# aleksgri/3D-wave-equation-MPI-CUDA

Hardware: AMD Instinct MI355X
Metric: Mpoints/sec (whole node) + L∞ error vs analytic, N=512³ fp64 (higher is better)
Workload: dtype fp64; 1 GPU; model=wave3d leapfrog 7-point, N=512^3, L=pi, T=1, timesteps=100, global_batch=1, seq_len=513, parallelism=dd1x1x1-tb4, N=512, kernel=tb4, overlap=False, overlap_mode=none, overlap_order=none, transport=self, hip_graph=True, device_bytes_per_gpu=4742168192

## Files before the change

3d-wave-equation-mpi-cuda_amd/csrc/hip_kernels.hip:

```cpp
#include <hip/hip_runtime.h>

#include <cstdlib>

#include <algorithm>

#include "device_common.hpp"


namespace wave3d {
namespace {

template <class T>
struct StepParams {
    int xcd;
    int delta;
    const T* u1;
    const T* u2;
    T* u;
    T* dout;
    i64 si;
    int sj;
    int poff;
    int jmax, kmax;
    int nbox;
// ... 342 lines not shown
    if (j <= bx.j1) {
        const T tyj = ty[j];
        bool nz = false, any = false;
        for (int i = ib; i <= ie; ++i) {
            const T txi = tx[i];
            const i64 row = i64(j) * sj;
            for (int k = bx.k0 + lane; k <= bx.k1; k += 64) {
                const T f = analytic(txi, tyj, tz[k], ct);
                u[i64(i) * si + row + k] = f;
#pragma unroll
                for (int q = 0; q < kMaxWrap; ++q)
                    if (i == wrap.src[q]) u[i64(wrap.dst[q]) * si + row + k] = f;
                chk += f;
                nz |= f != T(0);
                any = true;
            }
        }
        if (any) ma = T(0);
        if (nz) mr = T(0);
    }
    commit_errors(ma, mr, chk, err);
}

template <class T>
__global__ void k_zero_faces(T* u, i64 si, int sj, int X, int Y, int Z, int G, int mask) {
    const int i = 1 - G + blockIdx.y;
    const int t = 1 + blockIdx.x * blockDim.x + threadIdx.x;
    T* pl = u + i64(i) * si;
    if (t <= Y) {
        if (mask & 1) pl[t * sj + 1] = T(0);
        if (mask & 2) pl[t * sj + Z] = T(0);
    }
    if (t <= Z) {
        if (mask & 4) pl[1 * sj + t] = T(0);
        if (mask & 8) pl[Y * sj + t] = T(0);
    }
}

template <class T>
struct FaceOps {
    FaceOp<T> op[4];
};

template <class T>
__global__ void k_faces(T* u, i64 si, int sj, int ny, int nz, FaceOps<T> ops, bool to_buf) {
    const FaceOp<T> f = ops.op[blockIdx.z];
// ... 61 lines not shown
    return v.march && !v.flat ? kWaves * v.rows : kNaiveTJ;
}

int tile_order() {
    static const int order = [] {
        const char* e = std::getenv("WAVE3D_TILE_ORDER");
        const std::string v = e ? e : "";
        if (v == "k") return 0;
        if (v == "j") return 1;
        if (v == "blocks") return 3;
        W3D_REQUIRE(v.empty() || v == "band", "WAVE3D_TILE_ORDER must be band, blocks, j or k, not " + v);
        return 2;
    }();
    return order;
}

bool xcd_swizzle_enabled() {
    static const bool on = [] {
        const char* e = std::getenv("WAVE3D_XCD_SWIZZLE");
        return e && e[0] == '1';
    }();
    return on;
}

KernelVariant parse_kernel_variant(const std::string& name) {
    KernelVariant v;
    if (name == "naive") {
        v.march = false;
        return v;
    }
    if (name == "flat") {
        v.march = false, v.flat = true;
        return v;
    }
    if (name == "auto") {
        v.rows = 4;
        v.nt = true;
        return v;
    }
    W3D_REQUIRE(name.rfind("march", 0) == 0, "wave3d: unknown kernel variant " + name);
    std::string s = name.substr(5);
    if (!s.empty() && (s[0] == '2' || s[0] == '4' || s[0] == '8')) v.rows = s[0] - '0', s = s.substr(1);
    if (s == "nt") v.nt = true;
    else if (s == "f") v.fast = true;
    else if (s == "p") v.pk = true;
    else W3D_REQUIRE(s.empty(), "wave3d: unknown kernel variant " + name);
// ... 128 lines not shown
        L.block_begin = total;
        total += L.tiles_k * L.tiles_j * cdiv(planes, ch);
        ++nb;
    }
    p.nbox = nb;
    if (nb == 0) return;
    void (*kern)(const StepParams<T>);
    if (march) kern = first ? march_kernel<T, true>(kind) : march_kernel<T, false>(kind);
    else kern = first ? k_naive<T, true> : k_naive<T, false>;
    hipLaunchKernelGGL(kern, dim3(total), dim3(kThreads), 0, s, p);
    HIP_OK(hipGetLastError());
}

template <class T>
void launch_init(T* u, const GridView& gv, const Box& bx, const Wrap& wrap, const T* tx,
                 const T* ty, const T* tz, double ct0, u64* err, hipStream_t s) {
    if (bx.empty()) return;
    W3D_REQUIRE(bx.i0 >= 1 && bx.i1 <= gv.X && bx.j1 <= gv.Y && bx.k1 <= gv.Z,
                "init box outside the owned region");
    const int planes = bx.i1 - bx.i0 + 1;
    const int rowblocks = cdiv(bx.j1 - bx.j0 + 1, kWaves);
    const int chunk = std::min(planes, std::max(1, cdiv(planes * rowblocks, 4096)));
    dim3 grid(rowblocks, cdiv(planes, chunk));
    hipLaunchKernelGGL(k_init<T>, grid, dim3(kThreads), 0, s, u, gv.si, gv.sj, bx, chunk, wrap, tx,
                       ty, tz, T(ct0), err);
    HIP_OK(hipGetLastError());
}

template <class T>
void launch_zero_faces(T* u, const GridView& gv, int mask, hipStream_t s) {
    if (!mask) return;
    dim3 grid(cdiv(std::max(gv.Y, gv.Z), 256), gv.X + 2 * gv.G);
    hipLaunchKernelGGL(k_zero_faces<T>, grid, dim3(256), 0, s, u, gv.si, gv.sj, gv.X, gv.Y, gv.Z,
                       gv.G, mask);
    HIP_OK(hipGetLastError());
}

template <class T>
void launch_faces(T* u, const GridView& gv, const FaceOp<T>* ops, int nops, bool to_buf,
                  hipStream_t s) {
    W3D_REQUIRE(nops <= 4, "too many faces");
    if (nops <= 0) return;
    FaceOps<T> f{};
    for (int q = 0; q < nops; ++q) f.op[q] = ops[q];
    const int len = std::max(gv.Y, gv.Z) + 2;
    dim3 grid(cdiv(len, 256), gv.X, nops);
    hipLaunchKernelGGL(k_faces<T>, grid, dim3(256), 0, s, u, gv.si, gv.sj, gv.Y + 2, gv.Z + 2, f,
                       to_buf);
// ... 118 lines not shown
```

3d-wave-equation-mpi-cuda_amd/csrc/hip_kernels.hpp:

```cpp
#pragma once

#include <hip/hip_runtime.h>

#include <string>

#include "common.hpp"

namespace wave3d {

struct GridView {
    int X = 0, Y = 0, Z = 0;
    int G = 1;
    int sj = 0;
    i64 si = 0;
    int poff = 0;
    int jmax() const { return Y + G; }
    int kmax() const { return Z + G; }
};

constexpr int kMaxBoxes = 7;
constexpr int kTileK = 64;

struct StepCoefs {
    double hx2 = 1, hy2 = 1, hz2 = 1;
// ... 46 lines not shown
    int axis = 1;
    int index = 0;
};
template <class T>
void launch_faces(T* u, const GridView& gv, const FaceOp<T>* ops, int nops, bool to_buf,
                  hipStream_t s);

template <class T>
struct SeamPartners {
    int next_i = -(1 << 30), prev_i = -(1 << 30);
    const T *nA = nullptr, *nC = nullptr;
    const T *pA = nullptr, *pC = nullptr;
};
template <class T>
struct SeamCPlane {
    T* out = nullptr;
    const T *Ac = nullptr, *Am = nullptr, *Ap = nullptr, *Bc = nullptr;
    T* dout = nullptr;
};
constexpr int kMaxSeamOps = 6;
template <class T>
void launch_seam_c(bool first, bool delta, bool fm, const SeamCPlane<T>* ops, int nops, const GridView& gv,
                   const Box& cdom, const StepCoefs& cC, hipStream_t s);
bool tb3_supported(int rows, int waves, bool fm = false);
bool tb3_delta_supported(int rows, int waves, bool fm = false);
template <class T>
void launch_tb3(int rows, int waves, bool delta, bool fm, bool first, const T* A, const T* B, T* D, T* E,
                const GridView& gv, const Box* boxes, int nbox, const Box& cdom, int ei0, int ei1,
                const Wrap& wrapD, const Wrap& wrapE, const SeamPartners<T>& seam, const T* txy,
                const T* tz, const T* txr, const T* rtz, const StepCoefs& cC, const StepCoefs& cD,
                const StepCoefs& cE, u64* errC, u64* errD, u64* errE, int chunk, hipStream_t s);

constexpr int kTbnMaxDepth = 4;
template <class T>
struct TbnSeam {
    int next_i = -(1 << 30), prev_i = -(1 << 30);
    const T* nP[kTbnMaxDepth - 1] = {};
    const T* pP[kTbnMaxDepth - 1] = {};
};
bool tbn_supported(int depth, int rows, int waves, bool fm, bool fp32);
bool tbn_delta_supported(int depth, int rows, int waves, bool fm, bool fp32);
template <class T>
void launch_tbn(int depth, int rows, int waves, bool fm, bool first, const T* A, const T* B, T* O0, T* O1,
                const GridView& gv, const Box* boxes, int nbox, const Box& cdom, int ei0, int ei1,
                const Wrap& wrap0, const Wrap& wrap1, const TbnSeam<T>& seam, const T* txy, const T* tz,
                const T* txr, const T* rtz, const StepCoefs* c, u64* const* err, int chunk, hipStream_t s,
// ... 36 lines not shown
```

3d-wave-equation-mpi-cuda_amd/csrc/hip_solver.hip:

```cpp
#include <hip/hip_runtime.h>

#include <algorithm>
#include <chrono>
#include <cstdlib>
#include <cstring>
#include <iostream>
#include <map>
#include <memory>
#include <thread>

#include "checkpoint.hpp"
#include "device_common.hpp"
#include "hip_kernels.hpp"
#include "hip_selftest.hpp"
#include "rccl_transport.hpp"
#include "problem.hpp"
#include "sizing.hpp"
#include "solver.hpp"
#include "log.hpp"
#include "trace.hpp"

#define HIP_CHECK(x)                                                                   \
    do {                                                                               \
        hipError_t e_ = (x);                                                           \
// ... 62 lines not shown
        int peer, tag;
        int level;
        Box box;
        T* buf;
    };
    std::vector<BoxMsg> tb_bsends[2], tb_brecvs[2];
    std::vector<BoxMsg> tb_dsends, tb_drecvs;
    struct PeerBuf {
        int peer;
        T* buf;
        size_t count;
    };
    std::vector<PeerBuf> tb_psends, tb_precvs;
    struct PipeGroup {
        std::vector<PlaneMsg> sends, recvs;
        std::vector<BoxMsg> dsends, drecvs;
        std::vector<PeerBuf> psends, precvs;
    };
    std::vector<PipeGroup> pipe;
    std::vector<Box> slabs;
    T* alias[2][2] = {};
    T* seamc_buf = nullptr;
    T* seamc_in = nullptr;
    T* pinned = nullptr;
    Box tb_interior;
    std::vector<Box> tb_shell;
};

constexpr int kAliasPlane = -1000;

template <class T>
class HipSolver {
public:
    HipSolver(const Config& c, Transport* ext) : cfg_(c), ext_(ext) {
        prob_ = Problem::from_config(c);
        fault_ = FaultSpec::parse(c.fault);
        if (ext_) {
            W3D_REQUIRE(ext_->device(), "run_hip needs a device transport");
            world_ = ext_->size();
            local_ = {ext_->rank()};
        } else {
            world_ = std::max(1, c.ranks);
            for (int r = 0; r < world_; ++r) local_.push_back(r);
        }
        const Layout lay = plan_layout(c, world_);
        tb_ = lay.tb;
// ... 1035 lines not shown
            const T* cXp = op(c_ops, 2, Ap(X + 1), Ap(1), Ap(X + 2), Bp(X + 1));
            sp.next_i = 0, sp.nP[0] = Ap(X), sp.nP[1] = cX, sp.nP[2] = op(d_ops, 6, cX, cXm, cXp, dpl(8, Ap(X)));
            const T* c1 = op(c_ops, 3, Ap(1), Ap(0), Ap(2), Bp(1), 9);
            const T* c0 = op(c_ops, 4, Ap(0), Ap(-1), Ap(X), Bp(0));
            const T* c2 = op(c_ops, 5, Ap(2), Ap(1), Ap(3), Bp(2));
            sp.prev_i = X + 1, sp.pP[0] = Ap(1), sp.pP[1] = c1, sp.pP[2] = op(d_ops, 7, c1, c0, c2, dpl(9, Ap(1)));
        } else if (R.topo.first(0)) {
            const T* cN = op(c_ops, 0, aA, Ap(0), Ap(2), aB, 8);
            const T* cNm = op(c_ops, 1, Ap(0), Ap(-1), aA, Bp(0));
            const T* c1 = op(c_ops, 2, Ap(2), Ap(1), Ap(3), Bp(2));
            sp.next_i = 0, sp.nP[0] = aA, sp.nP[1] = cN, sp.nP[2] = op(d_ops, 6, cN, cNm, c1, dpl(8, aA));
        } else if (R.topo.last(0)) {
            const T* c0 = op(c_ops, 3, aA, Ap(X - 1), Ap(X + 1), aB, 9);
            const T* cm = op(c_ops, 4, Ap(X - 1), Ap(X - 2), Ap(X), Bp(X - 1));
            const T* cp = op(c_ops, 5, Ap(X + 1), aA, Ap(X + 2), Bp(X + 1));
            sp.prev_i = X + 1, sp.pP[0] = aA, sp.pP[1] = c0, sp.pP[2] = op(d_ops, 7, c0, cm, cp, dpl(9, aA));
        }
        return sp;
    }

    void seam4(DevRank<T>& R, int m, hipStream_t s) {
        std::vector<SeamCPlane<T>> c_ops, d_ops;
        seam_partners4(R, m, &c_ops, &d_ops);
        launch_seam_c<T>(m == 1, cfg_.delta, cfg_.fma, c_ops.data(), int(c_ops.size()), R.gv, R.cdom, coefs(m), s);
        launch_seam_c<T>(false, cfg_.delta, cfg_.fma, d_ops.data(), int(d_ops.size()), R.gv, R.cdom, coefs(m + 1), s);
    }

    void sweep4(DevRank<T>& R, int m, hipStream_t s, const Box* boxes = nullptr, int nbox = 0) {
        const T* A = R.g[lvl(m - 1)];
        const T* B = R.g[lvl(m - 2)];
        const TbnSeam<T> sp = seam_partners4(R, m, nullptr, nullptr);
        if (!boxes) boxes = &R.compute, nbox = 1;
        StepCoefs c[4];
        u64* err[4];
        for (int l = 0; l < 4; ++l) c[l] = coefs(m + l), err[l] = R.err + size_t(m + l) * kSlotsPerLayer;
        launch_tbn<T>(4, tb_rows_, tb_waves_, cfg_.fma, m == 1, A, B, R.g[lvl(m + 2)], R.g[lvl(m + 3)], R.gv, boxes,
                      nbox, R.cdom, R.error.i0, R.error.i1, R.wrap3, R.wrap4, sp, R.txy, R.tz, R.rtxy, R.rtz, c,
                      err, cfg_.chunk, s, cfg_.delta);
    }

    void seam_pre(DevRank<T>& R, int m, int span, hipStream_t s, bool in = false) {
        SeamScratch use(R, in);
        if (span == 4) seam4(R, m, s);
        else seam_c(R, m, s);
    }
    void sweep_deep(DevRank<T>& R, int m, int span, hipStream_t s, const Box* boxes = nullptr, int nbox = 0,
// ... 475 lines not shown
            launch_init<T>(R.g[lvl(0)], R.gv, R.owned, wrap_depth(R, G_), R.tx, R.ty, R.tz, ct_[0],
                           R.err, s_comp_);
            pack_faces(R, 0, s_comp_, true);
        }
        mark(s_comp_, 1);
        if (prob_.K >= 1) issue_exchange(0);
    }

    int enqueue_layers(RunResult& res, int start) {
        TraceRange tr("wave3d.layers");
        order_enqueued_ = !overlap_ ? "none" : pipe_ ? "pipe" : shells_first_ ? "shells_first" : "beside";
        pipe_prev_ = false;
        CuReserveScope cu_scope(s_comp_ == s_comp_cu_ ? comm_cus_ : 0);
        const int K = prob_.K;
        int done = start - 1;
        for (int n = start; n <= K;) {
            const int span = span_at(n);
            bool comm_follows = false;
            for (int q = n; q < n + span; ++q) guard_checkpoint_level(lvl(q), s_comp_);
            if (cfg_.delta && span == 1 && n > 1) guard_checkpoint_level(dlvl(n - 1), s_comp_);
            if (cfg_.print_layers && !cfg_.quiet && !capturing_ && ranks_[0].topo.rank == 0)
                for (int q = n; q < n + span; ++q) std::cout << "calculating layer " << q << "\n";
            mark(s_comp_, 0);
            for (int q = n; q < n + span; ++q)
                for (auto& R : ranks_)
                    if ((first_write_[q + 1] || q == start) && !(span >= 3 && q < n + span - 2))
                        launch_zero_faces<T>(R.g[lvl(q)], R.gv, R.zero_mask, s_comp_);
            bool exchanged = false;
            if (span >= 3 && overlap_ && pipe_) {
                pipe_sweep(n, span, n + span - 1 < K);
                exchanged = true;
            } else if (span >= 3 && overlap_ && shells_first_) {
                HIP_CHECK(hipStreamWaitEvent(s_comp_, ev_halo_, 0));
                for (auto& R : ranks_) {
                    seam_pre(R, n, span, s_comp_);
                    if (!R.tb_shell.empty())
                        sweep_deep(R, n, span, s_comp_, R.tb_shell.data(), int(R.tb_shell.size()));
                }
                const int last = n + span - 1;
                if (last < K) {
                    HIP_CHECK(hipEventRecord(ev_shell_, s_comp_));
                    HIP_CHECK(hipStreamWaitEvent(s_comm_, ev_shell_, 0));
                    issue_exchange(last, true);
                    exchanged = true;
                }
                for (auto& R : ranks_)
                    if (!R.tb_interior.empty()) sweep_deep(R, n, span, s_comp_, &R.tb_interior, 1);
            } else if (span >= 3 && overlap_) {
                HIP_CHECK(hipEventRecord(ev_layer_, s_comp_));
                HIP_CHECK(hipStreamWaitEvent(s_comm_, ev_layer_, 0));
// ... 428 lines not shown
```

3d-wave-equation-mpi-cuda_amd/csrc/hip_tb3.hip:

```cpp
#include <hip/hip_runtime.h>

#include <algorithm>
#include <climits>
#include <cmath>
#include <type_traits>

#include "device_common.hpp"

namespace wave3d {
namespace {

template <class T>
struct Tb3Params {
    const char* A;
    const char* B;
    char* D;
    char* E;
    unsigned pbytes;
    int pbias;
    int order;
    int sj;
    int poff;
    int jmin, jmax, kmin, kmax;
    int cj0, cj1, ck0, ck1;
// ... 540 lines not shown
    };
    commit_errors<T, NW>(ma1, rel(mr1, 0), chk1, p.errC);
    __syncthreads();
    commit_errors<T, NW>(ma2, rel(mr2, 1), chk2, p.errD);
    __syncthreads();
    commit_errors<T, NW>(ma3, rel(mr3, 2), chk3, p.errE);
}

template <class T>
struct SeamCOp {
    T* out;
    const T *Ac, *Am, *Ap, *Bc;
    T* dout;
};
template <class T>
struct SeamCParams {
    SeamCOp<T> op[kMaxSeamOps];
    int sj, jmin, jmax, kmin, kmax;
    int cj0, cj1, ck0, ck1;
    T hx2, hy2, hz2, yx2, yy2, yz2, coef;
    T fc[3];
};

template <class T, bool FIRST, bool DELTA, bool FM>
__global__ void __launch_bounds__(kThreads) k_seam_c(const SeamCParams<T> p) {
    const SeamCOp<T> o = p.op[blockIdx.y];
    const int ktiles = (p.kmax - p.kmin - 1 + kTK - 1) / kTK;
    const int j = p.jmin + 1 + (int(blockIdx.x) / ktiles) * kWaves + int(threadIdx.x >> 6);
    const int k = p.kmin + 1 + (int(blockIdx.x) % ktiles) * kTK + int(threadIdx.x & 63);
    if (j > p.jmax - 1 || k > p.kmax - 1) return;
    const i64 c = i64(j) * p.sj + k;
    T v = T(0), d = T(0);
    if (j >= p.cj0 && j <= p.cj1 && k >= p.ck0 && k <= p.ck1) {
        const T a = o.Ac[c];
        if constexpr (FM) {
            const T l = coef_lap_fma(a, o.Am[c], o.Ap[c], o.Ac[c - p.sj], o.Ac[c + p.sj], o.Ac[c - 1], o.Ac[c + 1],
                                     p.fc[0], p.fc[1], p.fc[2]);
            if constexpr (DELTA)
                d = FIRST ? l : o.Bc[c] + l, v = a + d;
            else if constexpr (FIRST)
                v = a + l;
            else
                v = leap_fm(a, o.Bc[c], o.Am[c], o.Ap[c], o.Ac[c - p.sj], o.Ac[c + p.sj], o.Ac[c - 1], o.Ac[c + 1],
                            p.fc[0], p.fc[1], p.fc[2], fm_kc(p.fc[0], p.fc[1], p.fc[2]));
        } else {
            const T lap = laplace7_cr(a, o.Am[c], o.Ap[c], o.Ac[c - p.sj], o.Ac[c + p.sj], o.Ac[c - 1],
                                      o.Ac[c + 1], p.hx2, p.hy2, p.hz2, p.yx2, p.yy2, p.yz2);
            if constexpr (DELTA)
                d = FIRST ? p.coef * lap : delta_incr(o.Bc[c], lap, p.coef), v = a + d;
            else
                v = FIRST ? taylor_first(a, lap, p.coef) : leapfrog(a, o.Bc[c], lap, p.coef);
        }
    }
    o.out[c] = v;
    if (DELTA && o.dout) o.dout[c] = d;
}

template <class T, bool F>
static void (*tb3_kernel(int rows, int waves, bool fm = false))(const Tb3Params<T>) {
    if (fm) {
        switch (rows * 100 + waves) {
            case 208: return k_tb3<T, F, 2, 8, false, true>;
            case 108: return k_tb3<T, F, 1, 8, false, true>;
            case 116: return k_tb3<T, F, 1, 16, false, true>;
            default: return nullptr;
        }
    }
    switch (rows * 100 + waves) {
        case 404: return k_tb3<T, F, 4, 4>;
        case 208: return k_tb3<T, F, 2, 8>;
        case 204: return k_tb3<T, F, 2, 4>;
        case 116: return k_tb3<T, F, 1, 16>;
        case 108: return k_tb3<T, F, 1, 8>;
        default: return nullptr;
    }
}

}
// ... 112 lines not shown
                   const Box& cdom, const StepCoefs& cC, hipStream_t s) {
    W3D_REQUIRE(nops >= 0 && nops <= kMaxSeamOps, "seam C: too many planes");
    if (nops == 0) return;
    SeamCParams<T> p{};
    for (int q = 0; q < nops; ++q)
        p.op[q] = SeamCOp<T>{ops[q].out, ops[q].Ac, ops[q].Am, ops[q].Ap, ops[q].Bc ? ops[q].Bc : ops[q].Ac, ops[q].dout};
    p.sj = gv.sj;
    p.jmin = 1 - gv.G, p.jmax = gv.jmax(), p.kmin = 1 - gv.G, p.kmax = gv.kmax();
    p.cj0 = cdom.j0, p.cj1 = cdom.j1, p.ck0 = cdom.k0, p.ck1 = cdom.k1;
    p.hx2 = T(cC.hx2), p.hy2 = T(cC.hy2), p.hz2 = T(cC.hz2);
    p.yx2 = T(1) / T(cC.hx2), p.yy2 = T(1) / T(cC.hy2), p.yz2 = T(1) / T(cC.hz2);
    p.coef = T(cC.coef);
    fma_coefs(cC, p.fc);
    const int rows = p.jmax - p.jmin - 1, ktiles = cdiv(p.kmax - p.kmin - 1, kTK);
    const dim3 grid(cdiv(rows, kWaves) * ktiles, nops);
    void (*kern)(const SeamCParams<T>) =
        fm ? (delta ? (first ? k_seam_c<T, true, true, true> : k_seam_c<T, false, true, true>)
                    : (first ? k_seam_c<T, true, false, true> : k_seam_c<T, false, false, true>))
           : (delta ? (first ? k_seam_c<T, true, true, false> : k_seam_c<T, false, true, false>)
                    : (first ? k_seam_c<T, true, false, false> : k_seam_c<T, false, false, false>));
    hipLaunchKernelGGL(kern, grid, dim3(kThreads), 0, s, p);
    HIP_OK(hipGetLastError());
}
template void launch_seam_c<double>(bool, bool, bool, const SeamCPlane<double>*, int, const GridView&, const Box&,
                                    const StepCoefs&, hipStream_t);
template void launch_seam_c<float>(bool, bool, bool, const SeamCPlane<float>*, int, const GridView&, const Box&,
                                   const StepCoefs&, hipStream_t);

#define W3D_TB3_INST(T)                                                                       \
    template void launch_tb3<T>(int, int, bool, bool, bool, const T*, const T*, T*, T*, const GridView&, \
                                const Box*, int, const Box&, int, int, const Wrap&,           \
                                const Wrap&, const SeamPartners<T>&, const T*,                \
                                const T*, const T*, const T*, const StepCoefs&, const StepCoefs&, \
                                const StepCoefs&, u64*, u64*, u64*, int, hipStream_t);
W3D_TB3_INST(double)
W3D_TB3_INST(float)

}
```

3d-wave-equation-mpi-cuda_amd/csrc/hip_tbn.hip:

```cpp
#include <hip/hip_runtime.h>

#include <algorithm>
#include <climits>
#include <cstdlib>
#include <cmath>
#include <type_traits>
#include <utility>

#include "device_common.hpp"

#ifndef W3D_TBN_ABL_ERR
#define W3D_TBN_ABL_ERR 0
#endif

#ifndef W3D_TBN_PART
#define W3D_TBN_PART 1
#endif
#ifndef W3D_TBN_BOUND
#define W3D_TBN_BOUND 0
#endif
#ifndef W3D_TBN_MERGE
#define W3D_TBN_MERGE 1
#endif
#ifndef W3D_TBN_PRE
#define W3D_TBN_PRE 1
#endif
#ifndef W3D_TBN_DENSE
#define W3D_TBN_DENSE 1
#endif

namespace wave3d {
template <class T>
const void* tbn_exact_kernel(int depth, bool first, bool delta);

namespace {

template <class F, int... I>
__device__ __forceinline__ void sfor_impl(F&& f, std::integer_sequence<int, I...>) {
    (f(std::integral_constant<int, I>{}), ...);
}
template <int N, class F>
__device__ __forceinline__ void sfor(F&& f) {
    sfor_impl(f, std::make_integer_sequence<int, N>{});
}
template <int V>
using Ic = std::integral_constant<int, V>;

template <class T>
struct TbnParams {
    const char* A;
    const char* B;
// ... 34 lines not shown
    static constexpr int scells = RPW * NW * W(0);
    static constexpr int bcells = RPW * NW * W(1);
    static constexpr int rowb = (kTK + 2 * D) * ES;
    static constexpr int browb = (kTK + 2 * D - 2) * ES;
    static constexpr int bat(int y, int x) { return y * W(1) + x - 1; }
    static constexpr int a_off(int q) { return q * scells; }
    static constexpr int b_off(int q) { return 4 * scells + q * bcells; }
    static constexpr int u_off(int s, int h) {
        return s == 1 ? b_off(2) + h * cells(1) : u_off(s - 1, 1) + cells(s - 1) + h * cells(s);
    }
    static constexpr int total = u_off(D - 1, 1) + cells(D - 1);
    static constexpr int npos(int r) {
        return 2 * (kTK + 2 * (r - 1)) + 2 * (TJ + 2 * (r - (r == D - 1 ? 1 : 0)));
    }
    static constexpr int first(int r) { return r <= 1 ? 0 : first(r - 1) + npos(r - 1); }
    static constexpr int ncomp = first(D);
    static constexpr int ring_of(int q) {
        int r = 1;
        while (r < D && q >= first(r + 1)) ++r;
        return r;
    }
};

template <int W, int ROWS, int NW>
struct DenseDma {
    static constexpr int pitch = W * 8, pay = pitch - 8;
    static constexpr int chunks = ((ROWS - 1) * pitch + pay + 15) / 16;
    static constexpr int PW = (chunks + 64 * NW - 1) / (64 * NW);
    static constexpr int NP = NW * PW;
    static constexpr int L = (chunks + NP - 1) / NP;
    static constexpr int last = chunks - (NP - 1) * L;
    static constexpr int src_row(int c) { return 16 * c / pitch + (16 * c % pitch == pay ? 1 : 0); }
    static constexpr int src_col(int c) { return 16 * c % pitch == pay ? -1 : 16 * c % pitch / 8; }
    static constexpr bool covers() {
        if (W % 2 == 0 || last < 1 || L > 64 || 2 * chunks < (ROWS - 1) * W + W - 1) return false;
        for (int c = 0; c < chunks; ++c)
            for (int h = 0; h < 2; ++h) {
                const int y = (2 * c + h) / W, x = (2 * c + h) % W;
                if (y >= ROWS) return false;
                if (x < W - 1 && (src_row(c) != y || src_col(c) + h != x)) return false;
            }
        return true;
    }
};
template <int D>
constexpr bool dense_dma_ok() {
    using Gm = TbnGeom<D, 16, 8, 8>;
    return DenseDma<Gm::W(0), Gm::H(0), 8>::covers() && DenseDma<Gm::W(1), Gm::H(0) - 2, 8>::covers();
}
static_assert(dense_dma_ok<4>() && dense_dma_ok<3>(), "dense LDS-DMA cover of the A / B frames");
static_assert(DenseDma<73, 24, 8>::chunks == 876 && DenseDma<71, 22, 8>::chunks == 781 && DenseDma<73, 24, 8>::PW == 2 &&
                  DenseDma<71, 22, 8>::PW == 2,
              "D = 4: 2 + 2 pieces per wave");

template <class T>
__device__ __forceinline__ unsigned lds_addr(T* ptr) {
    return static_cast<unsigned>(reinterpret_cast<uintptr_t>((__attribute__((address_space(3))) T*)ptr));
}
template <int ES, int ROWB, int RB>
__device__ __forceinline__ void dma_fill3(__amdgpu_buffer_rsrc_t r, unsigned src0, unsigned sjb, unsigned slot,
                                          unsigned lds0) {
    unsigned v0, v1, v2;
    u64 keep;
    const unsigned lane = __builtin_amdgcn_mbcnt_hi(~0u, __builtin_amdgcn_mbcnt_lo(~0u, 0u));
    if constexpr (ES == 8) {
        static_assert(RB % 16 == 0 && RB <= 1024, "fp64 rows: one dwordx4 piece per lane");
        asm volatile(
            "s_add_u32 m0, %[slot], %[lds0]\n\t"
            "v_add_u32 %[v0], %[src0], %[l16]\n\t"
            "v_add_u32 %[v1], %[sjb], %[v0]\n\t"
            "v_add_u32 %[v2], %[sjb], %[v1]\n\t"
            "s_mov_b64 %[keep], exec\n\t"
            "s_mov_b64 exec, %[mask]\n\t"
            "buffer_load_dwordx4 %[v0], %[rs], 0 offen lds\n\t"
            "s_add_u32 m0, m0, %[rowb]\n\t"
            "s_nop 0\n\t"
// ... 210 lines not shown
    unsigned ra_off[RP];
    bool rcd[RP];
    int ry[RP], rx[RP];
#pragma unroll
    for (int s = 0; s < RP; ++s) {
        const int q = threadIdx.x + s * NT;
        int g = 0, rj = jt, rk = kb;
#pragma unroll
        for (int d = 1; d < D; ++d)
            if (g == 0 && q < Gm::first(d + 1)) {
                g = d;
                ring(d, d == D - 1 ? 1 : 0, q - Gm::first(d), rj, rk);
            }
        rg[s] = g;
        ry[s] = rj - jt + D, rx[s] = rk - kb + D;
        ro0[s] = Gm::at(0, ry[s], rx[s]);
        rb0[s] = Gm::bat(ry[s], rx[s]);
        rcd[s] = g != 0 && incd(rj, rk);
        ra_off[s] = boff(rj, rk, g != 0 && inb(rj, rk));
    }

    constexpr bool DENSE = W3D_TBN_DENSE && ES == 8;
    using DA = DenseDma<W0, Gm::H(0), NW>;
    using DB = DenseDma<Gm::W(1), Gm::H(0) - 2, NW>;
    static_assert(DENSE || Gm::RPW == 3, "dma_fill3: three slot rows per wave");
    static_assert(!DENSE || (DA::PW == 2 && DB::PW == 2 && DA::covers() && DB::covers()),
                  "dma_dense2: two pieces per wave and fill");
    const unsigned sjb = unsigned(sj) * ES;
    const unsigned src0 = unsigned((jt - D + (DENSE ? 0 : w * Gm::RPW)) * sj + kb - D + p.poff) * ES;
    const unsigned lds0 = unsigned(DENSE ? w * 2 * DA::L * 16 : w * Gm::RPW * W0 * ES);
    const unsigned bds0 = unsigned(DENSE ? w * 2 * DB::L * 16 + Gm::W(1) * ES : w * Gm::RPW * Gm::W(1) * ES);
    auto dsrc = [&](auto geom, int q, unsigned origin) {
        using Dn = decltype(geom);
        const int c = min((w * Dn::PW + q) * Dn::L + lane, Dn::chunks - 1);
        return origin + unsigned(Dn::src_row(c)) * sjb + unsigned(Dn::src_col(c) * ES);
    };
    const unsigned da0 = DENSE ? dsrc(DA{}, 0, src0) : 0u, da1 = DENSE ? dsrc(DA{}, 1, src0) : 0u;
    const unsigned db0 = DENSE ? dsrc(DB{}, 0, src0 + sjb + ES) : 0u, db1 = DENSE ? dsrc(DB{}, 1, src0 + sjb + ES) : 0u;
    const unsigned nla = w == NW - 1 ? DA::last : DA::L, nlb = w == NW - 1 ? DB::last : DB::L;
    auto fillA = [&](auto qc, int plane, bool live) {
        const auto rs = prs(p.A, plane, live ? pbytes : 0u);
        if constexpr (DENSE) dma_dense2<DA::L, DA::L * 16>(rs, da0, da1, nla, lds_addr(Ap(qc)), lds0);
        else dma_fill3<ES, W0 * ES, Gm::rowb>(rs, src0, sjb, lds_addr(Ap(qc)), lds0);
    };
    auto fillB = [&](int q, int plane, bool live) {
        const auto rs = prs(p.B, plane, live ? pbytes : 0u);
        const unsigned slot = __builtin_amdgcn_readfirstlane(lds_addr(Bp(q)));
        if constexpr (DENSE) dma_dense2<DB::L, DB::L * 16>(rs, db0, db1, nlb, slot, bds0);
        else dma_fill3<ES, Gm::W(1) * ES, Gm::browb>(rs, src0 + ES, sjb, slot, bds0);
    };
    constexpr int NST = 2 * R;
    constexpr int PA = DENSE ? DA::PW : (ES == 8 ? 1 : 2) * Gm::RPW, PB = DENSE ? DB::PW : PA;
    constexpr bool PRE = W3D_TBN_PRE && ES == 8 && FM && !DELTA;
    constexpr int NPRE = std::min(2 + 3 * R + 5 * RP, 15);
    constexpr int NDMA = PA + (FIRST ? 0 : PB);
    fillA(Ic<3>{}, i0 - 1, true);
    fillA(Ic<0>{}, i0, true);
    fillA(Ic<1>{}, i0 + 1, true);
    fillA(Ic<2>{}, i0 + 2, true);
    if constexpr (!FIRST) fillB(0, i0, true);
    vm_wait<0>();
    __syncthreads();
// ... 512 lines not shown
```

Baseline: 624,900 Mpoints/s.

## Vectorize init kernel, fuse seam planes with face zeroing, rebalance B-frame DMA

Adds a 16-byte vectorized init kernel that caches tz values and writes whole vectors per lane. Adds a fused seam4 kernel that computes the layer-m seam planes and the layer-m+1 plane in one launch, using an LDS ring for neighbors, and folds the pending face-zeroing work into the same grid. Also changes the dense LDS-DMA split of the B frame so three waves load one piece and the rest load two. These changes aim to cut launch count and load imbalance, at the cost of redundant recomputation of layer-m values at tile halos and more complex indexing.

```diff
diff --git a/3d-wave-equation-mpi-cuda_amd/csrc/hip_kernels.hip b/3d-wave-equation-mpi-cuda_amd/csrc/hip_kernels.hip
--- a/3d-wave-equation-mpi-cuda_amd/csrc/hip_kernels.hip
+++ b/3d-wave-equation-mpi-cuda_amd/csrc/hip_kernels.hip
@@ -388,6 +388,76 @@
     commit_errors(ma, mr, chk, err);
 }
 
+constexpr int kInitQ = 5;
+constexpr int kInitRows = 64;
+template <class T>
+__global__ void __launch_bounds__(kThreads) k_init_wide(T* u, i64 si, int sj, Box bx, int ,
+                                                        Wrap wrap, const T* tx, const T* ty,
+                                                        const T* tz, T ct, u64* err) {
+    constexpr int W = 16 / int(sizeof(T));
+    typedef T VecT __attribute__((ext_vector_type(W)));
+    const int lane = threadIdx.x & 63, w = threadIdx.x >> 6;
+    const int i = bx.i0 + blockIdx.y;
+    const int jb = bx.j0 + blockIdx.x * kInitRows;
+    const int je = min(bx.j1, jb + kInitRows - 1);
+    const T txi = tx[i];
+    T* plane = u + i64(i) * si;
+    T ma = T(kErrInit), mr = T(kErrInit);
+    T chk = T(0);
+    bool nz = false, any = false;
+    const int g0 = (bx.k0 - 1) / W, g1 = (bx.k1 - 1) / W;
+    for (int gs = g0; gs <= g1; gs += 64 * kInitQ) {
+        T tzv[kInitQ][W];
+        int full = 0, part = 0;
+#pragma unroll
+        for (int q = 0; q < kInitQ; ++q) {
+            const int kb = 1 + (gs + q * 64 + lane) * W;
+#pragma unroll
+            for (int e = 0; e < W; ++e) {
+                const bool in = kb + e >= bx.k0 && kb + e <= bx.k1;
+                tzv[q][e] = in ? tz[kb + e] : T(0);
+                if (in) part |= 1 << q;
+            }
+            if (kb >= bx.k0 && kb + W - 1 <= bx.k1) full |= 1 << q;
+        }
+        for (int j = jb + w; j <= je; j += kWaves) {
+            const T tyj = ty[j];
+            T* row = plane + i64(j) * sj;
+            any |= part != 0;
+#pragma unroll
+            for (int q = 0; q < kInitQ; ++q) {
+                if (!(part >> q & 1)) continue;
+                const int kb = 1 + (gs + q * 64 + lane) * W;
+                VecT f;
+#pragma unroll
+                for (int e = 0; e < W; ++e) {
+                    f[e] = analytic(txi, tyj, tzv[q][e], ct);
+                    chk += f[e];
+                    nz |= f[e] != T(0);
+                }
+                if (full >> q & 1) {
+                    *reinterpret_cast<VecT*>(row + kb) = f;
+#pragma unroll
+                    for (int c = 0; c < kMaxWrap; ++c)
+                        if (i == wrap.src[c]) *reinterpret_cast<VecT*>(row + i64(wrap.dst[c] - i) * si + kb) = f;
+                } else {
+#pragma unroll
+                    for (int e = 0; e < W; ++e) {
+                        if (kb + e < bx.k0 || kb + e > bx.k1) continue;
+                        row[kb + e] = f[e];
+#pragma unroll
+                        for (int c = 0; c < kMaxWrap; ++c)
+                            if (i == wrap.src[c]) row[i64(wrap.dst[c] - i) * si + kb + e] = f[e];
+                    }
+                }
+            }
+        }
+    }
+    if (any) ma = T(0);
+    if (nz) mr = T(0);
+    commit_errors(ma, mr, chk, err);
+}
+
 template <class T>
 __global__ void k_zero_faces(T* u, i64 si, int sj, int X, int Y, int Z, int G, int mask) {
     const int i = 1 - G + blockIdx.y;
@@ -495,6 +565,13 @@
     }();
     return on;
 }
+
+static bool env_on(const char* key) {
+    const char* e = std::getenv(key);
+    return !(e && e[0] == '0');
+}
+bool init_wide_enabled() { return env_on("WAVE3D_INIT_WIDE"); }
+bool seam_fused_enabled() { return env_on("WAVE3D_SEAM_FUSED"); }
 
 KernelVariant parse_kernel_variant(const std::string& name) {
     KernelVariant v;
@@ -669,8 +746,12 @@
     const int rowblocks = cdiv(bx.j1 - bx.j0 + 1, kWaves);
     const int chunk = std::min(planes, std::max(1, cdiv(planes * rowblocks, 4096)));
     dim3 grid(rowblocks, cdiv(planes, chunk));
-    hipLaunchKernelGGL(k_init<T>, grid, dim3(kThreads), 0, s, u, gv.si, gv.sj, bx, chunk, wrap, tx,
-                       ty, tz, T(ct0), err);
+    constexpr int W = 16 / int(sizeof(T));
+    const bool wide = init_wide_enabled() && bx.k0 >= 1 && reinterpret_cast<uintptr_t>(u + 1) % 16 == 0 &&
+                      gv.sj % W == 0 && gv.si % W == 0;
+    if (wide) grid = dim3(cdiv(bx.j1 - bx.j0 + 1, kInitRows), planes);
+    hipLaunchKernelGGL(wide ? k_init_wide<T> : k_init<T>, grid, dim3(kThreads), 0, s, u, gv.si, gv.sj, bx,
+                       chunk, wrap, tx, ty, tz, T(ct0), err);
     HIP_OK(hipGetLastError());
 }
 
diff --git a/3d-wave-equation-mpi-cuda_amd/csrc/hip_kernels.hpp b/3d-wave-equation-mpi-cuda_amd/csrc/hip_kernels.hpp
--- a/3d-wave-equation-mpi-cuda_amd/csrc/hip_kernels.hpp
+++ b/3d-wave-equation-mpi-cuda_amd/csrc/hip_kernels.hpp
@@ -92,6 +92,12 @@
 template <class T>
 void launch_seam_c(bool first, bool delta, bool fm, const SeamCPlane<T>* ops, int nops, const GridView& gv,
                    const Box& cdom, const StepCoefs& cC, hipStream_t s);
+template <class T>
+void launch_seam4(bool first, bool delta, bool fm, const SeamCPlane<T>* c_ops, int nc, const SeamCPlane<T>* d_ops,
+                  int nd, T* const* faces, int nfaces, int mask, const GridView& gv, const Box& cdom,
+                  const StepCoefs& cC, const StepCoefs& cD, hipStream_t s);
+bool init_wide_enabled();
+bool seam_fused_enabled();
 bool tb3_supported(int rows, int waves, bool fm = false);
 bool tb3_delta_supported(int rows, int waves, bool fm = false);
 template <class T>
diff --git a/3d-wave-equation-mpi-cuda_amd/csrc/hip_solver.hip b/3d-wave-equation-mpi-cuda_amd/csrc/hip_solver.hip
--- a/3d-wave-equation-mpi-cuda_amd/csrc/hip_solver.hip
+++ b/3d-wave-equation-mpi-cuda_amd/csrc/hip_solver.hip
@@ -108,6 +108,7 @@
     T* alias[2][2] = {};
     T* seamc_buf = nullptr;
     T* seamc_in = nullptr;
+    std::vector<T*> face_pend;
     T* pinned = nullptr;
     Box tb_interior;
     std::vector<Box> tb_shell;
@@ -1189,6 +1190,14 @@
     void seam4(DevRank<T>& R, int m, hipStream_t s) {
         std::vector<SeamCPlane<T>> c_ops, d_ops;
         seam_partners4(R, m, &c_ops, &d_ops);
+        if (seam_fused_enabled()) {
+            launch_seam4<T>(m == 1, cfg_.delta, cfg_.fma, c_ops.data(), int(c_ops.size()), d_ops.data(),
+                            int(d_ops.size()), R.face_pend.data(), int(R.face_pend.size()), R.zero_mask, R.gv, R.cdom,
+                            coefs(m), coefs(m + 1), s);
+            R.face_pend.clear();
+            return;
+        }
+        W3D_REQUIRE(R.face_pend.empty(), "faces left to a pre-stage that does not clear them");
         launch_seam_c<T>(m == 1, cfg_.delta, cfg_.fma, c_ops.data(), int(c_ops.size()), R.gv, R.cdom, coefs(m), s);
         launch_seam_c<T>(false, cfg_.delta, cfg_.fma, d_ops.data(), int(d_ops.size()), R.gv, R.cdom, coefs(m + 1), s);
     }
@@ -1710,10 +1719,15 @@
             if (cfg_.print_layers && !cfg_.quiet && !capturing_ && ranks_[0].topo.rank == 0)
                 for (int q = n; q < n + span; ++q) std::cout << "calculating layer " << q << "\n";
             mark(s_comp_, 0);
+            const bool fuse_faces = span == 4 && !overlap_ && seam_fused_enabled();
             for (int q = n; q < n + span; ++q)
                 for (auto& R : ranks_)
-                    if ((first_write_[q + 1] || q == start) && !(span >= 3 && q < n + span - 2))
-                        launch_zero_faces<T>(R.g[lvl(q)], R.gv, R.zero_mask, s_comp_);
+                    if ((first_write_[q + 1] || q == start) && !(span >= 3 && q < n + span - 2)) {
+                        if (fuse_faces && R.zero_mask && (R.topo.dims[0] == 1 || R.topo.first(0) || R.topo.last(0)))
+                            R.face_pend.push_back(R.g[lvl(q)]);
+                        else
+                            launch_zero_faces<T>(R.g[lvl(q)], R.gv, R.zero_mask, s_comp_);
+                    }
             bool exchanged = false;
             if (span >= 3 && overlap_ && pipe_) {
                 pipe_sweep(n, span, n + span - 1 < K);
diff --git a/3d-wave-equation-mpi-cuda_amd/csrc/hip_tb3.hip b/3d-wave-equation-mpi-cuda_amd/csrc/hip_tb3.hip
--- a/3d-wave-equation-mpi-cuda_amd/csrc/hip_tb3.hip
+++ b/3d-wave-equation-mpi-cuda_amd/csrc/hip_tb3.hip
@@ -586,6 +586,32 @@
     T fc[3];
 };
 
+template <class T, bool FIRST, bool DELTA, bool FM, class P, class LoadB>
+__device__ __forceinline__ T seam_node(const P& p, T a, T xm, T xp, T jm, T jp, T km, T kp, LoadB bc, T& d) {
+    T v;
+    if constexpr (FM) {
+        if constexpr (DELTA || FIRST) {
+            const T l = coef_lap_fma(a, xm, xp, jm, jp, km, kp, p.fc[0], p.fc[1], p.fc[2]);
+            if constexpr (DELTA)
+                d = FIRST ? l : bc() + l, v = a + d;
+            else
+                v = a + l;
+        } else {
+            v = leap_fm(a, bc(), xm, xp, jm, jp, km, kp, p.fc[0], p.fc[1], p.fc[2],
+                        fm_kc(p.fc[0], p.fc[1], p.fc[2]));
+        }
+    } else {
+        const T lap = laplace7_cr(a, xm, xp, jm, jp, km, kp, p.hx2, p.hy2, p.hz2, p.yx2, p.yy2, p.yz2);
+        if constexpr (DELTA)
+            d = FIRST ? p.coef * lap : delta_incr(bc(), lap, p.coef), v = a + d;
+        else if constexpr (FIRST)
+            v = taylor_first(a, lap, p.coef);
+        else
+            v = leapfrog(a, bc(), lap, p.coef);
+    }
+    return v;
+}
+
 template <class T, bool FIRST, bool DELTA, bool FM>
 __global__ void __launch_bounds__(kThreads) k_seam_c(const SeamCParams<T> p) {
     const SeamCOp<T> o = p.op[blockIdx.y];
@@ -595,29 +621,94 @@
     if (j > p.jmax - 1 || k > p.kmax - 1) return;
     const i64 c = i64(j) * p.sj + k;
     T v = T(0), d = T(0);
-    if (j >= p.cj0 && j <= p.cj1 && k >= p.ck0 && k <= p.ck1) {
-        const T a = o.Ac[c];
-        if constexpr (FM) {
-            const T l = coef_lap_fma(a, o.Am[c], o.Ap[c], o.Ac[c - p.sj], o.Ac[c + p.sj], o.Ac[c - 1], o.Ac[c + 1],
-                                     p.fc[0], p.fc[1], p.fc[2]);
-            if constexpr (DELTA)
-                d = FIRST ? l : o.Bc[c] + l, v = a + d;
-            else if constexpr (FIRST)
-                v = a + l;
-            else
-                v = leap_fm(a, o.Bc[c], o.Am[c], o.Ap[c], o.Ac[c - p.sj], o.Ac[c + p.sj], o.Ac[c - 1], o.Ac[c + 1],
-                            p.fc[0], p.fc[1], p.fc[2], fm_kc(p.fc[0], p.fc[1], p.fc[2]));
-        } else {
-            const T lap = laplace7_cr(a, o.Am[c], o.Ap[c], o.Ac[c - p.sj], o.Ac[c + p.sj], o.Ac[c - 1],
-                                      o.Ac[c + 1], p.hx2, p.hy2, p.hz2, p.yx2, p.yy2, p.yz2);
-            if constexpr (DELTA)
-                d = FIRST ? p.coef * lap : delta_incr(o.Bc[c], lap, p.coef), v = a + d;
-            else
-                v = FIRST ? taylor_first(a, lap, p.coef) : leapfrog(a, o.Bc[c], lap, p.coef);
-        }
-    }
+    if (j >= p.cj0 && j <= p.cj1 && k >= p.ck0 && k <= p.ck1)
+        v = seam_node<T, FIRST, DELTA, FM>(p, o.Ac[c], o.Am[c], o.Ap[c], o.Ac[c - p.sj], o.Ac[c + p.sj], o.Ac[c - 1],
+                                           o.Ac[c + 1], [&] { return o.Bc[c]; }, d);
     o.out[c] = v;
     if (DELTA && o.dout) o.dout[c] = d;
+}
+
+template <class T>
+struct SeamCoef {
+    T hx2, hy2, hz2, yx2, yy2, yz2, coef;
+    T fc[3];
+};
+template <class T>
+struct Seam4Side {
+    SeamCOp<T> c, m, p;
+    T* outD;
+    const T* Bd;
+};
+template <class T>
+struct Seam4Params {
+    Seam4Side<T> side[2];
+    int nside, tiles;
+    int sj, jmin, jmax, kmin, kmax;
+    int cj0, cj1, ck0, ck1;
+    SeamCoef<T> cc, cd;
+    T* face[2];
+    i64 si;
+    int X, Y, Z, G, mask, fblocks;
+};
+
+template <class T, bool FIRST, bool DELTA, bool FM>
+__global__ void __launch_bounds__(kThreads) k_seam4(const Seam4Params<T> p) {
+    const int seam_blocks = p.nside * p.tiles;
+    if (int(blockIdx.x) >= seam_blocks) {
+        int b = int(blockIdx.x) - seam_blocks;
+        const int planes = p.X + 2 * p.G, per = p.fblocks * planes;
+        T* u = p.face[b / per];
+        b %= per;
+        T* pl = u + i64(1 - p.G + b / p.fblocks) * p.si;
+        const int t = 1 + (b % p.fblocks) * kThreads + int(threadIdx.x);
+        if (t <= p.Y) {
+            if (p.mask & 1) pl[t * p.sj + 1] = T(0);
+            if (p.mask & 2) pl[t * p.sj + p.Z] = T(0);
+        }
+        if (t <= p.Z) {
+            if (p.mask & 4) pl[1 * p.sj + t] = T(0);
+            if (p.mask & 8) pl[p.Y * p.sj + t] = T(0);
+        }
+        return;
+    }
+    const Seam4Side<T> o = p.side[int(blockIdx.x) / p.tiles];
+    const int tile = int(blockIdx.x) % p.tiles;
+    const int ktiles = (p.kmax - p.kmin - 1 + kTK - 1) / kTK;
+    const int jt = p.jmin + 1 + (tile / ktiles) * kWaves, kt = p.kmin + 1 + (tile % ktiles) * kTK;
+    __shared__ T ring[kWaves + 2][kTK + 2];
+    auto in_dom = [&](int j, int k) { return j >= p.cj0 && j <= p.cj1 && k >= p.ck0 && k <= p.ck1; };
+    auto layer_m = [&](const SeamCOp<T>& q, int j, int k, T& d) {
+        d = T(0);
+        if (!in_dom(j, k)) return T(0);
+        const i64 c = i64(j) * p.sj + k;
+        return seam_node<T, FIRST, DELTA, FM>(p.cc, q.Ac[c], q.Am[c], q.Ap[c], q.Ac[c - p.sj], q.Ac[c + p.sj],
+                                              q.Ac[c - 1], q.Ac[c + 1], [&] { return q.Bc[c]; }, d);
+    };
+    const int w = int(threadIdx.x >> 6), lane = int(threadIdx.x & 63);
+    const int j = jt + w, k = kt + lane;
+    T dc = T(0), dn;
+    const T vc = layer_m(o.c, j, k, dc);
+    ring[w + 1][lane + 1] = vc;
+    if (threadIdx.x < 2 * kTK) {
+        const int r = threadIdx.x < kTK ? 0 : kWaves + 1;
+        ring[r][lane + 1] = layer_m(o.c, jt - 1 + r, k, dn);
+    } else if (threadIdx.x < 2 * kTK + 2 * kWaves) {
+        const int q = int(threadIdx.x) - 2 * kTK, r = q >> 1, cc = (q & 1) * (kTK + 1);
+        ring[r + 1][cc] = layer_m(o.c, jt + r, kt - 1 + cc, dn);
+    }
+    __syncthreads();
+    if (j > p.jmax - 1 || k > p.kmax - 1) return;
+    const i64 c = i64(j) * p.sj + k;
+    T v = T(0), dd;
+    if (in_dom(j, k)) {
+        const T vm = layer_m(o.m, j, k, dn), vp = layer_m(o.p, j, k, dn);
+        v = seam_node<T, false, DELTA, FM>(p.cd, vc, vm, vp, ring[w][lane + 1], ring[w + 2][lane + 1],
+                                           ring[w + 1][lane], ring[w + 1][lane + 2],
+                                           [&] { return DELTA ? dc : o.Bd[c]; }, dd);
+    }
+    o.c.out[c] = vc;
+    if (DELTA && o.c.dout) o.c.dout[c] = dc;
+    o.outD[c] = v;
 }
 
 template <class T, bool F>
@@ -776,6 +867,67 @@
     hipLaunchKernelGGL(kern, grid, dim3(kThreads), 0, s, p);
     HIP_OK(hipGetLastError());
 }
+template <class T>
+static SeamCoef<T> seam_coef(const StepCoefs& c) {
+    SeamCoef<T> k{};
+    k.hx2 = T(c.hx2), k.hy2 = T(c.hy2), k.hz2 = T(c.hz2);
+    k.yx2 = T(1) / T(c.hx2), k.yy2 = T(1) / T(c.hy2), k.yz2 = T(1) / T(c.hz2);
+    k.coef = T(c.coef);
+    fma_coefs(c, k.fc);
+    return k;
+}
+
+template <class T>
+void launch_seam4(bool first, bool delta, bool fm, const SeamCPlane<T>* c_ops, int nc, const SeamCPlane<T>* d_ops,
+                  int nd, T* const* faces, int nfaces, int mask, const GridView& gv, const Box& cdom,
+                  const StepCoefs& cC, const StepCoefs& cD, hipStream_t s) {
+    W3D_REQUIRE(nd >= 0 && nd <= 2 && nc == 3 * nd, "seam4: three layer-m planes per layer-m+1 plane");
+    W3D_REQUIRE(nfaces >= 0 && nfaces <= 2, "seam4: at most two levels' faces");
+    if (!mask) nfaces = 0;
+    if (nd == 0 && nfaces == 0) return;
+    Seam4Params<T> p{};
+    auto cop = [&](const T* out) {
+        for (int q = 0; q < nc; ++q)
+            if (c_ops[q].out == out) {
+                const SeamCPlane<T>& o = c_ops[q];
+                return SeamCOp<T>{o.out, o.Ac, o.Am, o.Ap, o.Bc ? o.Bc : o.Ac, o.dout};
+            }
+        W3D_REQUIRE(false, "seam4: a layer-m+1 operand is no layer-m plane of this launch");
+        return SeamCOp<T>{};
+    };
+    for (int q = 0; q < nd; ++q) {
+        Seam4Side<T>& sd = p.side[q];
+        sd.c = cop(d_ops[q].Ac), sd.m = cop(d_ops[q].Am), sd.p = cop(d_ops[q].Ap);
+        sd.outD = d_ops[q].out;
+        sd.Bd = d_ops[q].Bc ? d_ops[q].Bc : d_ops[q].Ac;
+        W3D_REQUIRE(!d_ops[q].dout && !sd.m.dout && !sd.p.dout, "seam4: only the partner plane keeps its increment");
+        W3D_REQUIRE(!delta || (sd.c.dout && sd.Bd == sd.c.dout), "seam4: the increment of layer m is its own plane's");
+    }
+    p.nside = nd;
+    p.sj = gv.sj;
+    p.jmin = 1 - gv.G, p.jmax = gv.jmax(), p.kmin = 1 - gv.G, p.kmax = gv.kmax();
+    p.cj0 = cdom.j0, p.cj1 = cdom.j1, p.ck0 = cdom.k0, p.ck1 = cdom.k1;
+    p.cc = seam_coef<T>(cC), p.cd = seam_coef<T>(cD);
+    p.tiles = cdiv(p.jmax - p.jmin - 1, kWaves) * cdiv(p.kmax - p.kmin - 1, kTK);
+    for (int q = 0; q < nfaces; ++q) p.face[q] = faces[q];
+    p.si = gv.si, p.X = gv.X, p.Y = gv.Y, p.Z = gv.Z, p.G = gv.G, p.mask = mask;
+    p.fblocks = cdiv(std::max(gv.Y, gv.Z), kThreads);
+    const int total = p.nside * p.tiles + nfaces * p.fblocks * (gv.X + 2 * gv.G);
+    void (*kern)(const Seam4Params<T>) =
+        fm ? (delta ? (first ? k_seam4<T, true, true, true> : k_seam4<T, false, true, true>)
+                    : (first ? k_seam4<T, true, false, true> : k_seam4<T, false, false, true>))
+           : (delta ? (first ? k_seam4<T, true, true, false> : k_seam4<T, false, true, false>)
+                    : (first ? k_seam4<T, true, false, false> : k_seam4<T, false, false, false>));
+    hipLaunchKernelGGL(kern, dim3(total), dim3(kThreads), 0, s, p);
+    HIP_OK(hipGetLastError());
+}
+template void launch_seam4<double>(bool, bool, bool, const SeamCPlane<double>*, int, const SeamCPlane<double>*, int,
+                                   double* const*, int, int, const GridView&, const Box&, const StepCoefs&,
+                                   const StepCoefs&, hipStream_t);
+template void launch_seam4<float>(bool, bool, bool, const SeamCPlane<float>*, int, const SeamCPlane<float>*, int,
+                                  float* const*, int, int, const GridView&, const Box&, const StepCoefs&,
+                                  const StepCoefs&, hipStream_t);
+
 template void launch_seam_c<double>(bool, bool, bool, const SeamCPlane<double>*, int, const GridView&, const Box&,
                                     const StepCoefs&, hipStream_t);
 template void launch_seam_c<float>(bool, bool, bool, const SeamCPlane<float>*, int, const GridView&, const Box&,
diff --git a/3d-wave-equation-mpi-cuda_amd/csrc/hip_tbn.hip b/3d-wave-equation-mpi-cuda_amd/csrc/hip_tbn.hip
--- a/3d-wave-equation-mpi-cuda_amd/csrc/hip_tbn.hip
+++ b/3d-wave-equation-mpi-cuda_amd/csrc/hip_tbn.hip
@@ -27,6 +27,9 @@
 #endif
 #ifndef W3D_TBN_DENSE
 #define W3D_TBN_DENSE 1
+#endif
+#ifndef W3D_TBN_BDEAL
+#define W3D_TBN_BDEAL 1
 #endif
 
 namespace wave3d {
@@ -107,18 +110,23 @@
     }
 };
 
-template <int W, int ROWS, int NW>
+template <int W, int ROWS, int NW, int SOLO = 0>
 struct DenseDma {
     static constexpr int pitch = W * 8, pay = pitch - 8;
     static constexpr int chunks = ((ROWS - 1) * pitch + pay + 15) / 16;
     static constexpr int PW = (chunks + 64 * NW - 1) / (64 * NW);
-    static constexpr int NP = NW * PW;
+    static constexpr int NP = NW * PW - SOLO;
     static constexpr int L = (chunks + NP - 1) / NP;
     static constexpr int last = chunks - (NP - 1) * L;
+    static constexpr int count(int w) { return w < SOLO ? 1 : PW; }
+    static constexpr int first(int w) { return w < SOLO ? w : SOLO + (w - SOLO) * PW; }
     static constexpr int src_row(int c) { return 16 * c / pitch + (16 * c % pitch == pay ? 1 : 0); }
     static constexpr int src_col(int c) { return 16 * c % pitch == pay ? -1 : 16 * c % pitch / 8; }
     static constexpr bool covers() {
         if (W % 2 == 0 || last < 1 || L > 64 || 2 * chunks < (ROWS - 1) * W + W - 1) return false;
+        if (SOLO < 0 || SOLO >= NW || (SOLO > 0 && PW < 2) || first(0) != 0) return false;
+        for (int w = 0; w < NW; ++w)
+            if (count(w) < 1 || first(w) + count(w) != (w + 1 < NW ? first(w + 1) : NP)) return false;
         for (int c = 0; c < chunks; ++c)
             for (int h = 0; h < 2; ++h) {
                 const int y = (2 * c + h) / W, x = (2 * c + h) % W;
@@ -131,12 +139,16 @@
 template <int D>
 constexpr bool dense_dma_ok() {
     using Gm = TbnGeom<D, 16, 8, 8>;
-    return DenseDma<Gm::W(0), Gm::H(0), 8>::covers() && DenseDma<Gm::W(1), Gm::H(0) - 2, 8>::covers();
+    return DenseDma<Gm::W(0), Gm::H(0), 8>::covers() && DenseDma<Gm::W(1), Gm::H(0) - 2, 8>::covers() &&
+           DenseDma<Gm::W(1), Gm::H(0) - 2, 8, 3>::covers() && DenseDma<Gm::W(1), Gm::H(0) - 2, 8, 3>::L < 64;
 }
 static_assert(dense_dma_ok<4>() && dense_dma_ok<3>(), "dense LDS-DMA cover of the A / B frames");
 static_assert(DenseDma<73, 24, 8>::chunks == 876 && DenseDma<71, 22, 8>::chunks == 781 && DenseDma<73, 24, 8>::PW == 2 &&
                   DenseDma<71, 22, 8>::PW == 2,
               "D = 4: 2 + 2 pieces per wave");
+static_assert(DenseDma<71, 22, 8, 3>::NP == 13 && DenseDma<71, 22, 8, 3>::L == 61 && DenseDma<71, 22, 8, 3>::last == 49 &&
+                  DenseDma<71, 22, 8, 3>::first(7) == 11,
+              "D = 4, B dealt by ring load: 3 x 1 + 5 x 2 pieces");
 
 template <class T>
 __device__ __forceinline__ unsigned lds_addr(T* ptr) {
@@ -393,22 +405,23 @@
 
     constexpr bool DENSE = W3D_TBN_DENSE && ES == 8;
     using DA = DenseDma<W0, Gm::H(0), NW>;
-    using DB = DenseDma<Gm::W(1), Gm::H(0) - 2, NW>;
+    using DB = DenseDma<Gm::W(1), Gm::H(0) - 2, NW, W3D_TBN_BDEAL ? 3 : 0>;
     static_assert(DENSE || Gm::RPW == 3, "dma_fill3: three slot rows per wave");
     static_assert(!DENSE || (DA::PW == 2 && DB::PW == 2 && DA::covers() && DB::covers()),
                   "dma_dense2: two pieces per wave and fill");
     const unsigned sjb = unsigned(sj) * ES;
     const unsigned src0 = unsigned((jt - D + (DENSE ? 0 : w * Gm::RPW)) * sj + kb - D + p.poff) * ES;
     const unsigned lds0 = unsigned(DENSE ? w * 2 * DA::L * 16 : w * Gm::RPW * W0 * ES);
-    const unsigned bds0 = unsigned(DENSE ? w * 2 * DB::L * 16 + Gm::W(1) * ES : w * Gm::RPW * Gm::W(1) * ES);
+    const unsigned bds0 = unsigned(DENSE ? DB::first(w) * DB::L * 16 + Gm::W(1) * ES : w * Gm::RPW * Gm::W(1) * ES);
     auto dsrc = [&](auto geom, int q, unsigned origin) {
         using Dn = decltype(geom);
-        const int c = min((w * Dn::PW + q) * Dn::L + lane, Dn::chunks - 1);
+        const int c = min((Dn::first(w) + q) * Dn::L + lane, Dn::chunks - 1);
         return origin + unsigned(Dn::src_row(c)) * sjb + unsigned(Dn::src_col(c) * ES);
     };
     const unsigned da0 = DENSE ? dsrc(DA{}, 0, src0) : 0u, da1 = DENSE ? dsrc(DA{}, 1, src0) : 0u;
     const unsigned db0 = DENSE ? dsrc(DB{}, 0, src0 + sjb + ES) : 0u, db1 = DENSE ? dsrc(DB{}, 1, src0 + sjb + ES) : 0u;
-    const unsigned nla = w == NW - 1 ? DA::last : DA::L, nlb = w == NW - 1 ? DB::last : DB::L;
+    const unsigned nla = w == NW - 1 ? DA::last : DA::L;
+    const unsigned nlb = DB::count(w) < 2 ? 0 : w == NW - 1 ? DB::last : DB::L;
     auto fillA = [&](auto qc, int plane, bool live) {
         const auto rs = prs(p.A, plane, live ? pbytes : 0u);
         if constexpr (DENSE) dma_dense2<DA::L, DA::L * 16>(rs, da0, da1, nla, lds_addr(Ap(qc)), lds0);
```

Result: no change. 630,800 Mpoints/s (median of 6 runs) (+0.9%).
